# honglu2875/hironaka

Hardware: NVIDIA B200
Metric: game_steps_per_sec (higher is better)
Workload: dtype int32

## Files before the change

### hironaka_b200/csrc/hk_capi.cu

```cuda
#include <cuda_runtime.h>

#include <atomic>
#include <cstdio>
#include <cstring>
#include <new>

#include "hk_experience.cuh"
#include "hk_launch.cuh"
#include "hk_value.cuh"

using hk::StepParams;
using hk::kMaxDevices;

namespace hk {
int launch_small_i32_noobs(const StepParams& p, int dev, cudaStream_t stream);
int launch_small_i32_obs(const StepParams& p, int dev, cudaStream_t stream);
int launch_small_f32_noobs(const StepParams& p, int dev, cudaStream_t stream);
int launch_small_f32_obs(const StepParams& p, int dev, cudaStream_t stream);
int launch_small_i32(const StepParams& p, bool obs, int dev, cudaStream_t stream) {
    return obs ? launch_small_i32_obs(p, dev, stream) : launch_small_i32_noobs(p, dev, stream);
}
int launch_small_f32(const StepParams& p, bool obs, int dev, cudaStream_t stream) {
    return obs ? launch_small_f32_obs(p, dev, stream) : launch_small_f32_noobs(p, dev, stream);
}
// ... 48 lines not shown
        if (nibble && (p.d > 3 || !(p.flags & HK_F_ACT_DISCRETE))) return HK_ERR_BAD_ARG;
        if (host_fixed) p.host_action = nullptr;
        if (agent_fixed || packed) p.axis = nullptr;
        if ((p.ops & HK_OP_SHIFT) &&
            ((!host_fixed && p.host_action == nullptr) || (!agent_fixed && !packed && p.axis == nullptr)))
            return HK_ERR_BAD_ARG;
    }
    if ((p.ops & HK_OP_RESCALE) && dtype != HK_DTYPE_F32) return HK_ERR_UNSUPPORTED;
    if (p.ops & ~(HK_OP_SHIFT | HK_OP_REPOSITION | HK_OP_NEWTON | HK_OP_RESCALE | HK_OP_DEDUPE)) return HK_ERR_BAD_ARG;
    {
        const uint32_t sm = p.flags & (HK_F_OBS_SORT_COORD0 | HK_F_OBS_SORT_LEX | HK_F_OBS_SORT_LEX_FIRST);
        if (sm & (sm - 1)) return HK_ERR_BAD_ARG;
    }
    if (p.T < 1) return HK_ERR_BAD_ARG;
    if (p.B == 0) return HK_OK;
    int dev = 0;
    cudaError_t e = cudaGetDevice(&dev);
    if (e != cudaSuccess) return (int)e;
    const bool obs = p.obs != nullptr;
    if (p.done_bits && !p.census) return HK_ERR_UNSUPPORTED;
    if (p.census) {
        const bool policy = p.flags & (HK_F_HOST_ALL_COORD | HK_F_HOST_ZEILLINGER | HK_F_AGENT_FIRST | HK_F_AGENT_LAST);
        if (p.out != p.in || p.T != 1 || policy || p.host_out || p.ops == 0) return HK_ERR_UNSUPPORTED;
        const bool sched = hk::is_small_shape(p.N, p.d) && !force_generic && !(p.ops & HK_OP_DEDUPE);
        if (obs && !(sched && (p.flags & (HK_F_OBS_SORT_COORD0 | HK_F_OBS_SORT_LEX | HK_F_OBS_SORT_LEX_FIRST))))
            return HK_ERR_UNSUPPORTED;
        if (sched && obs)
            return dtype == HK_DTYPE_I32 ? hk::launch_sched_i32_obs(p, dev, stream) : hk::launch_sched_f32_obs(p, dev, stream);
        if (sched)
            return dtype == HK_DTYPE_I32 ? hk::launch_sched_i32(p, dev, stream) : hk::launch_sched_f32(p, dev, stream);
        if (hk::rows_shape(p.N, p.d) && !(p.ops & HK_OP_DEDUPE) && !g_no_rows_kernel.load()) {
            p.live_mask = reinterpret_cast<uint64_t*>(p.census + ((p.B + 7) & ~7ll));
            int rc2 = dtype == HK_DTYPE_I32 ? hk::launch_rows_i32(p, dev, stream) : hk::launch_rows_f32(p, dev, stream);
            if (rc2 != HK_OK) return rc2;
            p.rows_k = hk::ROWS_K;
        } else if (p.done_bits) {
            e = cudaMemsetAsync(p.done_bits, 0, (size_t)((p.B + 31) / 32) * 4, stream);
            if (e != cudaSuccess) return (int)e;
        }
        return dtype == HK_DTYPE_I32 ? hk::launch_generic_i32(p, false, dev, stream) : hk::launch_generic_f32(p, false, dev, stream);
    }
    const bool small = hk::is_small_shape(p.N, p.d) && !force_generic && !(p.ops & HK_OP_DEDUPE);
    if (dtype == HK_DTYPE_I32)
        return small ? hk::launch_small_i32(p, obs, dev, stream) : hk::launch_generic_i32(p, obs, dev, stream);
    return small ? hk::launch_small_f32(p, obs, dev, stream) : hk::launch_generic_f32(p, obs, dev, stream);
}

StepParams make_params(const void* in, void* out, long long B, int N, int d, float pad) {
    StepParams p;
    memset(&p, 0, sizeof(p));
    p.in = in;
    p.out = out;
    p.B = B;
    p.N = N;
    p.d = d;
// ... 3 lines not shown
    return p;
}

std::atomic<int> g_force_generic{0};
std::atomic<int> g_no_session_graphs{0};

}

namespace hk {
int device_sms(int dev) { return device_sms_impl(dev); }
bool use_pdl() { return g_use_pdl.load(std::memory_order_relaxed) != 0; }
int sched_geometry() { return g_sched_geometry.load(std::memory_order_relaxed); }
}

extern "C" {

int hk_version(void) { return HK_VERSION; }

const char* hk_error_string(int code) {
    switch (code) {
        case HK_OK: return "ok";
        case HK_ERR_BAD_ARG: return "bad argument (null pointer, non-positive size or bad flag combination)";
        case HK_ERR_UNSUPPORTED: return "unsupported shape or op for this dtype";
        case HK_ERR_ALIGN: return "state pointer is not 4-byte aligned";
        default: return code > 0 ? cudaGetErrorString((cudaError_t)code) : "unknown error";
    }
}

int hk_kernel_class(int N, int d) {
    if (check_shape(1, N, d, HK_DTYPE_I32) != HK_OK) return HK_ERR_UNSUPPORTED;
    return (hk::is_small_shape(N, d) && !g_force_generic.load()) ? 1 : 0;
}

int hk_debug_set_pdl(int on) {
    g_use_pdl.store(on ? 1 : 0);
    return HK_OK;
}

int hk_debug_set_sched_geometry(int which) {
    g_sched_geometry.store(which);
    return HK_OK;
}

int hk_debug_set_rows_kernel(int on) {
    g_no_rows_kernel.store(on ? 0 : 1);
    return HK_OK;
}

int64_t hk_census_bytes(int64_t B, int32_t N, int32_t d) {
    if (B < 0) return 0;
    if (hk::is_small_shape(N, d) || !hk::rows_shape(N, d)) return B;
    return ((B + 7) & ~7ll) + 8 * B;
}

int hk_debug_set_session_graphs(int on) {
    g_no_session_graphs.store(on ? 0 : 1);
    return HK_OK;
}

int hk_debug_force_generic(int on) {
    g_force_generic.store(on ? 1 : 0);
    return HK_OK;
}

int hk_step(const void* state_in, void* state_out, const int32_t* host_action, const int32_t* axis, uint8_t* done,
            float* reward, int32_t* num_points, float* obs, const int32_t* obs_coord, int32_t* exceed_flag,
            int64_t B, int32_t N, int32_t d, int32_t dtype, uint32_t ops, uint32_t flags, float padding_value,
            float value_threshold, void* stream) {
    StepParams p = make_params(state_in, state_out, B, N, d, padding_value);
    p.host_action = host_action;
    p.axis = axis;
    p.done = done;
    p.reward = reward;
    p.num_points = num_points;
    p.obs = obs;
// ... 626 lines not shown
```

### hironaka_b200/csrc/hk_launch.cuh

```cuda
#pragma once
#include <cuda_runtime.h>

#include <atomic>
#include <cstring>

#include "hk_common.cuh"

namespace hk {

constexpr int kMaxDevices = 64;

int device_sms(int dev);
bool use_pdl();
int sched_geometry();

struct KernelFacts {
    std::atomic<int> ctas_per_sm[kMaxDevices];
    KernelFacts() {
        for (auto& c : ctas_per_sm) c.store(0);
    }
};

template <typename K>
int kernel_ctas_per_sm(K kernel, KernelFacts& facts, int dev, int threads, size_t smem, cudaError_t* err) {
// ... 6 lines not shown
    }
    e = cudaOccupancyMaxActiveBlocksPerMultiprocessor(&v, kernel, threads, smem);
    if (e != cudaSuccess) {
        *err = e;
        return 0;
    }
    if (v < 1) v = 1;
    facts.ctas_per_sm[dev].store(v, std::memory_order_release);
    return v;
}

inline bool is_small_shape(int N, int d) { return d == 3 && (N == 20 || N == 10 || N == 5); }

int launch_small_i32(const StepParams& p, bool obs, int dev, cudaStream_t stream);
int launch_small_f32(const StepParams& p, bool obs, int dev, cudaStream_t stream);
int launch_sched_i32(const StepParams& p, int dev, cudaStream_t stream);
int launch_sched_f32(const StepParams& p, int dev, cudaStream_t stream);
int launch_sched_i32_obs(const StepParams& p, int dev, cudaStream_t stream);
int launch_sched_f32_obs(const StepParams& p, int dev, cudaStream_t stream);
int launch_rows_i32(const StepParams& p, int dev, cudaStream_t stream);
int launch_rows_f32(const StepParams& p, int dev, cudaStream_t stream);
constexpr int ROWS_K = 8;
inline bool rows_shape(int N, int d) { return N <= 64 && d >= 2 && d <= 5; }
int launch_generic_i32(const StepParams& p, bool obs, int dev, cudaStream_t stream);
int launch_generic_f32(const StepParams& p, bool obs, int dev, cudaStream_t stream);

}
```

### hironaka_b200/csrc/hk_rows.cuh

```cuda
#pragma once
#include "hk_launch.cuh"
#include "hk_small.cuh"

namespace hk {

constexpr int ROWS_MAX_K = ROWS_K;
constexpr int ROWS_ROUND_GAMES = 1024;

template <int D, int WARPS, int STAGES>
struct RowsLayout {
    static constexpr int LANE_WORDS = ROWS_MAX_K * D + 1 - ((ROWS_MAX_K * D) & 1);
    static constexpr int STAGE_WORDS = 32 * LANE_WORDS;
    static constexpr int CLS_WORDS = ROWS_ROUND_GAMES / 4;
    static constexpr int ORDER_WORDS = ROWS_ROUND_GAMES / 2;
    static constexpr int WARP_WORDS = STAGES * STAGE_WORDS + CLS_WORDS + ORDER_WORDS;
    static constexpr size_t SMEM_BYTES = (size_t)WARPS * WARP_WORDS * 4;
};

__device__ __forceinline__ int census_count(uint32_t v) { return (v & 0x80u) ? (int)(v & 1u) : (int)v; }

template <typename T, int D, int K>
__device__ __forceinline__ void rows_step(const StepParams& p, const uint32_t* area, uint32_t* g_state, long long g,
                                          uint64_t mask, int cnt, bool valid, int32_t ha, int32_t ax, int& new_cnt,
                                          uint64_t& new_mask, bool& origin, bool& exceed) {
    T y[K * D];
    uint32_t clm = 0;
#pragma unroll
    for (int k = 0; k < K; ++k) {
        const bool lv = valid && k < cnt;
        clm |= lv ? (1u << k) : 0u;
#pragma unroll
        for (int c = 0; c < D; ++c) y[k * D + c] = lv ? Elem<T>::from_bits(area[k * D + c]) : Elem<T>::zero();
    }
    const uint32_t clm0 = clm;
    clm = game_step<T, K, D, 0, false>(y, clm, p.ops, p.flags, ha, ax);
    new_cnt = __popc(clm);
    if (p.exceed_flag) exceed = exceeds<T, K, D>(y, clm, p.threshold);
    const T padv = Elem<T>::pad(p.pad);
    uint64_t m = mask, nm = mask;
    uint32_t nz = 0;
#pragma unroll
    for (int k = 0; k < K; ++k) {
        if ((clm0 >> k) & 1u) {
            const int slot = __ffsll((long long)m) - 1;
            m &= m - 1;
            const bool alive = (clm >> k) & 1u;
            bool moved = false;
#pragma unroll
            for (int c = 0; c < D; ++c) {
                moved = moved || ((uint32_t)Elem<T>::bits(y[k * D + c]) != area[k * D + c]);
                nz |= alive ? (uint32_t)Elem<T>::bits(y[k * D + c]) : 0u;
            }
            if (!alive) nm &= ~(1ull << slot);
            if (!alive || moved) {
                uint32_t* dst = g_state + slot * D;
#pragma unroll
                for (int c = 0; c < D; ++c) dst[c] = (uint32_t)Elem<T>::bits(alive ? y[k * D + c] : padv);
            }
        }
    }
    new_mask = nm;
    origin = (nz == 0);
}

template <typename T, int D, int WARPS, int STAGES>
__global__ void __launch_bounds__(WARPS * 32) hk_rows_kernel(const StepParams p) {
    using L = RowsLayout<D, WARPS, STAGES>;
    constexpr int LW = L::LANE_WORDS;
    extern __shared__ __align__(128) uint8_t smem_raw[];
    const int warp = threadIdx.x >> 5, lane = threadIdx.x & 31;
    uint32_t* wbase = reinterpret_cast<uint32_t*>(smem_raw) + (size_t)warp * L::WARP_WORDS;
    uint32_t* stages = wbase;
    uint8_t* clsb = reinterpret_cast<uint8_t*>(wbase + STAGES * L::STAGE_WORDS);
    uint16_t* order = reinterpret_cast<uint16_t*>(wbase + STAGES * L::STAGE_WORDS + L::CLS_WORDS);

    const long long B = p.B;
    const int W = p.N * D;
    const long long gw = (long long)blockIdx.x * WARPS + warp;
    const long long nw = (long long)gridDim.x * WARPS;
    uint32_t* gst = reinterpret_cast<uint32_t*>(p.out);
    const uint32_t lt = (1u << lane) - 1u;
    const bool frozen_rest = (p.flags & HK_F_FREEZE_ENDED) && !(p.ops & (HK_OP_REPOSITION | HK_OP_RESCALE));
    const float rest_reward = (p.flags & HK_F_ROLE_AGENT) ? -0.0f : 0.0f;
    int done_total = 0;

    long long per = (B + nw - 1) / nw;
// ... 52 lines not shown
                total += __popc(bal);
            }
        }
        __syncwarp();
        const int nchunks = (total + 31) >> 5;

        struct Pick {
            long long g;
            uint64_t mask;
            int cnt;
            bool valid;
        };
        auto pick = [&](int v) -> Pick {
            Pick k;
            const int idx = v * 32 + lane;
            k.valid = idx < total;
            const int o = k.valid ? (int)order[idx] : 0;
            k.g = g0 + o;
            k.cnt = k.valid ? (int)(clsb[o] >> 2) : 0;
            k.mask = k.valid ? __ldg(reinterpret_cast<const unsigned long long*>(p.live_mask) + k.g) : 0ull;
            return k;
        };
        auto gather = [&](const Pick& k, uint32_t* stage) {
            uint32_t* area = stage + lane * LW;
            const uint32_t* src = gst + k.g * W;
            uint64_t m = k.mask;
#pragma unroll
            for (int r = 0; r < ROWS_MAX_K; ++r) {
                if (r < k.cnt) {
                    const int slot = __ffsll((long long)m) - 1;
                    m &= m - 1;
#pragma unroll
                    for (int c = 0; c < D; ++c) cp_async_4(area + r * D + c, src + slot * D + c);
                }
            }
            cp_async_commit();
        };

        Pick cur = pick(0), nxt;
        nxt.g = 0, nxt.mask = 0, nxt.cnt = 0, nxt.valid = false;
        gather(cur, stages);
        for (int v = 0; v < nchunks; ++v) {
            uint32_t* stage = stages + (STAGES == 1 ? 0 : (v & 1)) * L::STAGE_WORDS;
            int32_t ha = 3, ax = 0;
            if ((p.ops & HK_OP_SHIFT) && cur.valid) load_actions(p, p.flags, cur.g, 0, ha, ax);
            if (STAGES >= 2 && v + 1 < nchunks) {
                nxt = pick(v + 1);
                gather(nxt, stages + ((v + 1) & 1) * L::STAGE_WORDS);
                cp_async_wait<1>();
            } else {
                cp_async_wait<0>();
            }
            __syncwarp();
            const int cmax = __reduce_max_sync(0xffffffffu, cur.cnt);
            const uint32_t* area = stage + lane * LW;
            int ncnt = 0;
            uint64_t nmask = 0;
            bool origin = false, exceed = false;
            const bool prev_done = cur.cnt < 2;
// ... 35 lines not shown
```

### hironaka_b200/csrc/hk_sched.cuh

```cuda
#pragma once
#include "hk_small.cuh"

namespace hk {

constexpr int SCHED_ROUND_TILES = 32;
#ifndef SCHED_PASS_UNROLL
#define SCHED_PASS_UNROLL 2
#endif
constexpr int kSchedPassUnroll = SCHED_PASS_UNROLL;
#ifndef SCHED_TILE_GROUP
#define SCHED_TILE_GROUP 0
#endif
#ifndef SCHED_DIRECT
#define SCHED_DIRECT 1
#endif
#ifndef SCHED_SPECULATE
#define SCHED_SPECULATE 0
#endif
#ifndef SCHED_NATURAL_NUM
#define SCHED_NATURAL_NUM 1
#define SCHED_NATURAL_DEN 2
#endif

template <int N, int D, int WARPS, int STAGES, bool OBS = false>
struct SchedLayout {
    static constexpr int W = N * D;
    static constexpr int STAGE_WORDS = 32 * W;
    static constexpr int OBS_WORDS = OBS ? 32 * (W + D) : 0;
    static constexpr int CLS_WORDS = SCHED_ROUND_TILES * 32 / 4;
    static constexpr int ORDER_WORDS = SCHED_ROUND_TILES * 32 / 2;
    static constexpr int WARP_WORDS = STAGES * STAGE_WORDS + CLS_WORDS + ORDER_WORDS + OBS_WORDS;
    static constexpr int BAR_BYTES = 256;
    static_assert(WARPS * STAGES * 8 <= BAR_BYTES, "mbarrier area too small");
    static constexpr size_t SMEM_BYTES = BAR_BYTES + (size_t)WARPS * WARP_WORDS * 4;
};

__device__ __forceinline__ int census_class(uint32_t v) {
    if (v == 0) return 6;
    if (v & 0x80u) return 1;
    return v <= 2 ? 1 : (v <= 4 ? 2 : (v <= 8 ? 3 : (v <= 12 ? 4 : (v <= 16 ? 5 : 6))));
}

template <typename T, int N, int D, int WARPS, int STAGES, bool OBS = false, int MINB = 1>
__global__ void __launch_bounds__(WARPS * 32, MINB) hk_sched_kernel(const StepParams p) {
    using L = SchedLayout<N, D, WARPS, STAGES, OBS>;
    constexpr int W = L::W;
    constexpr int CHW = (W % 4 == 0) ? 4 : ((W % 2 == 0) ? 2 : 1);
    constexpr int LPG = W / CHW;
    static_assert(LPG <= 32, "a game is copied by at most one warp instruction");
    constexpr int GPI = 32 / LPG;
    constexpr int COPY_ITERS = (32 + GPI - 1) / GPI;
    extern __shared__ __align__(128) uint8_t smem_raw[];
    const int warp = threadIdx.x >> 5, lane = threadIdx.x & 31;
    uint64_t* bar = reinterpret_cast<uint64_t*>(smem_raw) + warp * STAGES;
    uint32_t* wbase = reinterpret_cast<uint32_t*>(smem_raw + L::BAR_BYTES) + (size_t)warp * L::WARP_WORDS;
    uint32_t* stages = wbase;
    uint8_t* clsb = reinterpret_cast<uint8_t*>(wbase + STAGES * L::STAGE_WORDS);
    uint16_t* order = reinterpret_cast<uint16_t*>(wbase + STAGES * L::STAGE_WORDS + L::CLS_WORDS);
    float* obs_tile = reinterpret_cast<float*>(wbase + STAGES * L::STAGE_WORDS + L::CLS_WORDS + L::ORDER_WORDS);
    const int OW = W + (p.obs_coord ? D : 0);
    const bool obs_bulk = OBS && aligned16(p.obs) && ((OW & 3) == 0);

    const long long B = p.B;
    const long long ntiles = (B + 31) >> 5;
    const long long gw = (long long)blockIdx.x * WARPS + warp;
    const long long nw = (long long)gridDim.x * WARPS;
    uint32_t* gst = reinterpret_cast<uint32_t*>(p.out);
    const bool piece_ok = ((reinterpret_cast<uintptr_t>(p.out)) & (CHW * 4 - 1)) == 0;
    const bool bulk = ((W * 4) % 16 == 0) && aligned16(p.out);
    if (lane == 0) {
#pragma unroll
        for (int s = 0; s < STAGES; ++s) mbar_init(&bar[s], 1);
        mbar_fence_init();
    }
    __syncwarp();
    uint32_t phase_bits = 0;
    const uint32_t lt = (1u << lane) - 1u;
    const bool frozen_rest = (p.flags & HK_F_FREEZE_ENDED) && !(p.ops & (HK_OP_REPOSITION | HK_OP_RESCALE));
    const float rest_reward = (p.flags & HK_F_ROLE_AGENT) ? -0.0f : 0.0f;
    const int sub = lane / LPG, piece = lane - sub * LPG;
    int settled_total = 0;

// ... 63 lines not shown
                    fence_async_smem();
                    __syncwarp();
                    if (lane == 0) {
                        mbar_expect_tx(&bar[0], (uint32_t)__popc(vbal) * (uint32_t)(W * 4));
                        bulk_load(stages, gst + first * W, (uint32_t)__popc(vbal) * (uint32_t)(W * 4), &bar[0]);
                    }
                }
            }
            if constexpr (!OBS) {
                if (rest) {
                    if (p.done) p.done[g] = 1;
                    if (p.reward) p.reward[g] = rest_reward;
                    if (p.num_points) p.num_points[g] = (int32_t)(v & 1u);
                }
                const uint32_t restmask = __ballot_sync(0xffffffffu, rest);
                settled_total += __popc(restmask);
                if (p.done_bits && lane == 0) p.done_bits[tile_of(j0 + k)] = restmask;
            }
        }
        classes = __reduce_or_sync(0xffffffffu, classes) & ~1u;
        const bool natural = OBS ? (inplay * 4 >= ngames) : (inplay * SCHED_NATURAL_DEN >= ngames * SCHED_NATURAL_NUM);
        __syncwarp();
        int total = 0;
        if (!natural && inplay <= 32) {
#pragma unroll kSchedPassUnroll
            for (int k = 0; k < nk; ++k) {
                if (!((tilemask >> k) & 1u)) continue;
                const bool m = (clsb[k * 32 + lane] & 7u) != 0u;
                const uint32_t bal = __ballot_sync(0xffffffffu, m);
                if (m) order[total + __popc(bal & lt)] = (uint16_t)(k * 32 + lane);
                total += __popc(bal);
            }
        }
        for (int q = 1; q <= 6 && !natural && inplay > 32; ++q) {
            if (!((classes >> q) & 1u)) continue;
            for (int k = 0; k < nk; ++k) {
                if (!((tilemask >> k) & 1u)) continue;
                const bool m = (clsb[k * 32 + lane] & 7u) == (uint32_t)q;
                const uint32_t bal = __ballot_sync(0xffffffffu, m);
                if (m) order[total + __popc(bal & lt)] = (uint16_t)(k * 32 + lane);
                total += __popc(bal);
            }
        }
        __syncwarp();
        const int nchunks = natural ? __popc(tilemask) : ((total + 31) >> 5);
        uint32_t tiles_left = tilemask;

        auto chunk_game = [&](int v, long long& g, bool& valid) {
            if (natural) {
                const int k = __ffs((int)tiles_left) - 1;
                tiles_left &= tiles_left - 1;
                g = (tile_of(j0 + k) << 5) + lane;
                valid = (g < B) && ((clsb[k * 32 + lane] & 7u) != 0);
                return;
            }
            const int idx = v * 32 + lane;
            valid = idx < total;
// ... 40 lines not shown
                for (int it = 0; it < COPY_ITERS; ++it) {
                    const int s = it * GPI + sub;
                    const long long gs = __shfl_sync(0xffffffffu, g, s & 31);
                    const bool vs = __shfl_sync(0xffffffffu, valid ? 1 : 0, s & 31) != 0;
                    if (sub < GPI && s < 32 && vs) {
                        uint32_t* dst = stage + s * W + piece * CHW;
                        const uint32_t* src = gst + gs * W + piece * CHW;
                        if constexpr (CHW == 4) cp_async_16(dst, src);
                        else if constexpr (CHW == 2) cp_async_8(dst, src);
                        else cp_async_4(dst, src);
                    }
                }
            } else {
                for (int s = 0; s < 32; ++s) {
                    const long long gs = __shfl_sync(0xffffffffu, g, s);
                    const bool vs = __shfl_sync(0xffffffffu, valid ? 1 : 0, s) != 0;
                    if (vs) {
                        for (int w = lane; w < W; w += 32) cp_async_4(stage + s * W + w, gst + gs * W + w);
                    }
                }
            }
            cp_async_commit();
        };

        long long g_cur = 0, g_nxt = 0;
        bool v_cur = false, v_nxt = false;
        if (spec && !natural) {
            mbar_wait(&bar[0], phase_bits & 1u);
            phase_bits ^= 1u;
            spec = false;
        }
        if (inplay) {
            chunk_game(0, g_cur, v_cur);
            if (!spec) gather(g_cur, v_cur, stages, 0);
        }
        for (int k = 0; OBS && k < nk; ++k) {
            const long long g = (tile_of(j0 + k) << 5) + lane;
            const uint32_t code = clsb[k * 32 + lane];
            const bool rest = code & 0x80u;
            const uint32_t v = (code >> 6) & 1u;
            if (rest) {
                if (p.done) p.done[g] = 1;
                if (p.reward) p.reward[g] = rest_reward;
                if (p.num_points) p.num_points[g] = (int32_t)v;
            }
            const uint32_t restmask = __ballot_sync(0xffffffffu, rest);
            settled_total += __popc(restmask);
            if constexpr (OBS) {
                if (p.obs && restmask && !(natural && ((tilemask >> k) & 1u))) {
                    float* orow = obs_tile + lane * OW;
                    bulk_wait_read<0>();
                    __syncwarp();
                    if (rest) {
                        const float z = (v & 1u) ? 0.0f : p.pad;
                        const uint32_t ocm = p.obs_coord ? action_mask(load_action(p.obs_coord, g, p.flags), p.flags) : 0u;
                        if ((OW & 3) == 0 && D <= 4 && !p.obs_coord) {
                            float4* o4 = reinterpret_cast<float4*>(orow);
// ... 26 lines not shown
                            m &= m - 1;
                            warp_copy_words(reinterpret_cast<uint32_t*>(p.obs + (first + r) * OW),
                                            reinterpret_cast<uint32_t*>(obs_tile + r * OW), OW, lane);
                        }
                    }
                    __syncwarp();
                }
            }
            if (p.done_bits && lane == 0) p.done_bits[tile_of(j0 + k)] = restmask;
        }
        __syncwarp();
        if (inplay == 0) continue;
        for (int v = 0; v < nchunks; ++v) {
            const int sidx = (STAGES == 1) ? 0 : (v & 1);
            uint32_t* stage = stages + sidx * L::STAGE_WORDS;
            LaneState ls;
            ls.g = g_cur;
            ls.valid = v_cur;
            ls.shift = (p.ops & HK_OP_SHIFT) && ls.valid;
            ls.ha = 3;
            ls.ax = 0;
            ls.origin = false;
            if (ls.shift) load_actions(p, p.flags, ls.g, 0, ls.ha, ls.ax);
            if constexpr (STAGES == 1 && HK_L2_PREFETCH) {
                if (bulk && natural && tiles_left && lane == 0) {
                    const long long tn = tile_of(j0 + (__ffs((int)tiles_left) - 1));
                    const long long left = B - (tn << 5);
                    bulk_prefetch_l2(gst + (tn << 5) * W, (uint32_t)(left < 32 ? left : 32) * (uint32_t)(W * 4));
                }
            }
            if (bulk) {
                mbar_wait(&bar[sidx], (phase_bits >> sidx) & 1u);
                phase_bits ^= (1u << sidx);
            }
            if constexpr (STAGES >= 2) {
                if (v + 1 < nchunks) {
                    chunk_game(v + 1, g_nxt, v_nxt);
                    gather(g_nxt, v_nxt, stages + ((v + 1) & 1) * L::STAGE_WORDS, (v + 1) & 1);
                    if (!bulk) cp_async_wait<1>();
                } else {
                    if (!bulk) cp_async_wait<0>();
                }
            } else {
                if (!bulk) cp_async_wait<0>();
            }
            __syncwarp();
// ... 1 lines not shown
            bool exceed = false;
            bool chg = false;
            bool released = false;
            if constexpr (SCHED_DIRECT && !OBS && STAGES == 1 && !Elem<T>::is_float) {
                auto release = [&]() {
                    released = true;
                    __syncwarp();
                    if (v + 1 < nchunks) {
                        chunk_game(v + 1, g_nxt, v_nxt);
                        gather(g_nxt, v_nxt, stages, 0);
                    }
                };
                small_process_tile<T, N, D, false, true, decltype(release)>(p, ls, row, exceed, chg, gst + ls.g * W,
                                                                            release);
            } else {
                small_process_tile<T, N, D, false>(p, ls, row, exceed, chg);
            }
            if (ls.valid) {
                if (p.num_points) p.num_points[ls.g] = ls.cnt;
                if (p.done_bits && ls.cnt < 2) atomicOr(p.done_bits + (ls.g >> 5), 1u << (ls.g & 31));
                const uint32_t nv = (ls.cnt <= 1) ? (0x80u | (ls.origin ? 2u : 0u) | (uint32_t)ls.cnt)
                                                  : (uint32_t)(ls.cnt > 127 ? 127 : ls.cnt);
                p.census[ls.g] = (uint8_t)nv;
            }
            if (p.exceed_flag) {
                if (__any_sync(0xffffffffu, exceed && ls.valid) && lane == 0) *p.exceed_flag = 1;
            }
            if constexpr (OBS) {
                if (p.obs) {
                    const bool ingrid = ls.g < B;
                    float* orow = obs_tile + lane * OW;
                    bulk_wait_read<0>();
                    __syncwarp();
                    {
                        T z[W];
                        load_game<T, W>(row, z);
                        if constexpr (Elem<T>::is_float) {
#pragma unroll
                            for (int q = 0; q < W; ++q) z[q] = z[q] + 0.0f;
                        }
                        const uint32_t zl = live_mask<T, N, D>(z);
                        const int zmax = __reduce_max_sync(0xffffffffu, ingrid ? __popc(zl) : 0);
                        bool built = false;
                        if constexpr (D <= 6) built = features_network<T, N, D>(z, zl, zmax, p.flags, p.pad, orow);
                        if (!built) {
                            const int gpow = (OW & -OW) > 32 ? 32 : (OW & -OW);
// ... 103 lines not shown
```

### hironaka_b200/csrc/hk_small.cuh

```cuda
#pragma once
#include <type_traits>

#include "hk_common.cuh"

namespace hk {

constexpr int SMALL_BAR_BYTES = 256;
#ifndef HK_SPARSE_STORE_MAX
#define HK_SPARSE_STORE_MAX 16
#endif

template <int N, int D, bool OBS, int WARPS, int STAGES>
struct SmallLayout {
    static_assert(WARPS * STAGES * 8 <= SMALL_BAR_BYTES, "mbarrier area too small");
    static constexpr int W = N * D;
    static constexpr int TILE_WORDS = 32 * W;
    static constexpr int OBS_W = W + D;
    static constexpr int OBS_WORDS = OBS ? 32 * OBS_W : 0;
    static constexpr int WARP_WORDS = STAGES * TILE_WORDS + OBS_WORDS;
    static constexpr size_t SMEM_BYTES = SMALL_BAR_BYTES + (size_t)WARPS * WARP_WORDS * 4;
};

template <typename T, int W>
__device__ __forceinline__ void load_game(const uint32_t* s, T (&x)[W]) {
// ... 283 lines not shown
            lm = op_newton<T, N, D>(x, lm);
        }
    }
    if constexpr (Elem<T>::is_float) {
        if (ops & HK_OP_RESCALE) op_rescale<N, D>(x, lm, flags & HK_F_RESCALE_EPS);
    }
    return lm;
}

template <typename T>
__device__ __forceinline__ T x_row_value(const uint32_t* row, int w) {
    T v = Elem<T>::from_bits(row[w]);
    if constexpr (Elem<T>::is_float) v = v + 0.0f;
    return v;
}

struct LaneState {
    long long g;
    bool valid, shift;
    int32_t ha, ax;
    int cnt;
    int32_t len;
    bool origin;
};

__host__ __device__ constexpr int next_lower_tier(int K) {
    return K > 16 ? 16 : (K > 12 ? 12 : (K > 8 ? 8 : (K > 4 ? 4 : 0)));
}

template <typename T, int N, int D, int K, bool POLICY>
__device__ __forceinline__ int tier_steps(const StepParams& p, LaneState& ls, uint32_t* row, uint32_t lm, int st,
                                          bool& exceed, bool& chg) {
    const long long B = p.B;
    const T padv = Elem<T>::pad(p.pad);
    const bool mutate = p.ops != 0;
    constexpr bool ROLLED = (K >= 12) && (K < N) && ((N * D) % 4 == 0);
    constexpr int RS = !ROLLED ? 0 : ((D == 3 && 4 * K <= N * D) ? 4 : D);
    constexpr int LOWER = next_lower_tier(K);
    T y[K * D];
    int idx[K];
    uint32_t clm = 0, cvalid = 0;
    if constexpr (K == N) {
        load_game<T, N * D>(row, y);
        if constexpr (Elem<T>::is_float) {
#pragma unroll
            for (int q = 0; q < N * D; ++q) y[q] = y[q] + 0.0f;
// ... 37 lines not shown
        if (ls.valid) {
            if (p.done) p.done[(long long)st * B + ls.g] = dn ? 1 : 0;
            if (p.reward) {
                float r = (dn && !prev_done) ? 1.0f : 0.0f;
                p.reward[(long long)st * B + ls.g] = (p.flags & HK_F_ROLE_AGENT) ? -r : r;
            }
        }
        if (p.done_count) {
            const int c = __popc(__ballot_sync(0xffffffffu, ls.valid && dn));
            if ((threadIdx.x & 31) == 0 && c) atomicAdd(p.done_count + st, c);
        }
        if (dn && !prev_done) ls.len = st + 1;
        ls.ha = ha_n;
        ls.ax = ax_n;
        ++st;
        if constexpr (LOWER > 0) {
            if (st < p.T && __reduce_max_sync(0xffffffffu, ls.valid ? ls.cnt : 0) <= LOWER) break;
        }
    }
    chg = tchg;
    const bool last = st >= p.T;
    if (last && p.exceed_flag) exceed = exceeds<T, K, D>(y, clm, p.threshold);
    if (p.census) {
        if (K <= 4 || __any_sync(0xffffffffu, ls.cnt <= 1)) {
            uint32_t nz = 0;
#pragma unroll
            for (int k = 0; k < K; ++k) {
                uint32_t o = 0;
#pragma unroll
                for (int c = 0; c < D; ++c) o |= (uint32_t)Elem<T>::bits(y[k * D + c]);
                nz |= ((clm >> k) & 1u) ? o : 0u;
            }
            ls.origin = (nz == 0);
        } else {
            ls.origin = false;
        }
    }
    if (mutate) {
        if constexpr (K == N) {
#pragma unroll
            for (int i = 0; i < N; ++i) {
#pragma unroll
                for (int c = 0; c < D; ++c) y[i * D + c] = ((clm >> i) & 1u) ? y[i * D + c] : padv;
            }
            store_game<T, N * D>(row, y);
        } else {
// ... 51 lines not shown
        k[i] = min(a_, b_);                  \
        k[j] = max(a_, b_);                  \
    }
#include "hk_sortnet.inc"
#undef HK_CE
}

template <int D>
struct PackedRow {
    static constexpr int FB = 27 / D;
    static constexpr uint32_t VMAX = (1u << (FB - 1)) - 1u;
    static constexpr uint32_t FMASK = (1u << FB) - 1u;
    __host__ __device__ static constexpr uint32_t guards() {
        uint32_t g = 0;
        for (int c = 0; c < D; ++c) g |= 1u << (5 + FB * c + FB - 1);
        return g;
    }
};

struct NoRelease {
    __device__ __forceinline__ void operator()() const {}
};

template <int N, int D, int K, bool DIRECT = false, typename Release = NoRelease>
__device__ __forceinline__ bool tier_packed(const StepParams& p, LaneState& ls, uint32_t* row, uint32_t lm_in, int lmax, int st,
                                            bool& exceed, bool& chg, uint32_t* gdst = nullptr, Release release = Release()) {
    using P = PackedRow<D>;
    constexpr uint32_t G = P::guards();
    const uint32_t lm = ls.valid ? lm_in : 0u;
    const int cnt0 = __popc(lm);
    uint32_t M[D], csel[D];
    const int ax = ls.ax;
    bool apply = false;
    {
        uint32_t cm = 0;
        if (p.ops & HK_OP_SHIFT) {
            cm = action_mask(ls.ha, p.flags);
            apply = (ax >= 0) && (ax < D);
            if (p.flags & HK_F_NOOP_INVALID) apply = apply && ((cm >> (ax & 31)) & 1u);
            if (p.flags & HK_F_FREEZE_ENDED) apply = apply && (cnt0 >= 2);
        }
        const uint32_t into = apply ? (1u << (5 + P::FB * ax)) : 0u;
#pragma unroll
        for (int c = 0; c < D; ++c) {
            csel[c] = apply ? ((cm >> c) & 1u) : 0u;
            M[c] = ((apply && c == ax) ? 0u : (1u << (5 + P::FB * c))) + csel[c] * into;
        }
    }
    constexpr int KLOW = (K > 16) ? 16 : ((K > 12) ? 12 : (K > 8 ? 8 : (K > 4 ? 4 : 0)));
    uint32_t w[K];
    uint32_t uor = 0, orig0 = 0, orig_hi = 0;
    uint32_t mn[D], mns = 0xffffffffu;
#pragma unroll
    for (int c = 0; c < D; ++c) mn[c] = 0xffffffffu;
    {
        uint32_t m = lm;
        int i = 0;
        uint32_t pa[D], ps = 0xffffffffu;
#pragma unroll
        for (int c = 0; c < D; ++c) pa[c] = 0xffffffffu;
#pragma unroll
        for (int k = 0; k < K; ++k) {
            if (k >= KLOW && k >= lmax) {
                w[k] = 0xffffffffu;
                continue;
            }
            const bool v = m != 0;
            i = v ? (__ffs((int)m) - 1) : i;
            m &= m - 1;
            uint32_t a[D];
#pragma unroll
            for (int c = 0; c < D; ++c) a[c] = row[i * D + c];
            if (k == 0) {
#pragma unroll
                for (int c = 0; c < D; ++c) {
                    orig0 += a[c] << (5 + P::FB * c);
                    orig_hi |= a[c];
                }
            }
            uint32_t q = (uint32_t)i, sum = 0;
#pragma unroll
            for (int c = 0; c < D; ++c) {
                q += a[c] * M[c];
                sum += a[c] * csel[c];
                uor |= a[c];
            }
            uor |= sum;
            if (k & 1) {
#pragma unroll
                for (int c = 0; c < D; ++c) mn[c] = __vimin3_u32(mn[c], pa[c], a[c]);
                mns = __vimin3_u32(mns, ps, sum);
            } else {
#pragma unroll
                for (int c = 0; c < D; ++c) pa[c] = a[c];
                ps = sum;
// ... 26 lines not shown
            for (int a = 0; a + 1 < b; a += 2) acc = __vimin3_u32(acc, ~(pb - w[a]) & G, ~(pb - w[a + 1]) & G);
            if (b & 1) acc = min(acc, ~(pb - w[b - 1]) & G);
            kill |= (acc == 0u) ? (1u << b) : 0u;
        }
    }
    const uint32_t live0 = (cnt0 >= 32) ? 0xffffffffu : ((1u << cnt0) - 1u);
    const uint32_t alive = live0 & ~kill;
    const int cnt = __popc(alive);
    const bool prev_done = cnt0 < 2, dn = cnt < 2;
    if (ls.valid) {
        if (p.done) p.done[(long long)st * p.B + ls.g] = dn ? 1 : 0;
        if (p.reward) {
            const float r = (dn && !prev_done) ? 1.0f : 0.0f;
            p.reward[(long long)st * p.B + ls.g] = (p.flags & HK_F_ROLE_AGENT) ? -r : r;
        }
    }
    if (p.done_count) {
        const int c = __popc(__ballot_sync(0xffffffffu, ls.valid && dn));
        if ((threadIdx.x & 31) == 0 && c) atomicAdd(p.done_count + st, c);
    }
    if (dn && !prev_done) ls.len = st + 1;
    ls.cnt = cnt;
    ls.origin = (cnt == 0) || (cnt == 1 && (w[0] >> 5) == 0u);
    const bool gchg = (cnt0 >= 2) || (cnt0 == 1 && lone_moved);
    if constexpr (!DIRECT) chg = chg || gchg;
    if (p.exceed_flag && st + 1 >= p.T) {
        uint32_t hi = 0;
#pragma unroll
        for (int b = 0; b < K; ++b) {
#pragma unroll
            for (int c = 0; c < D; ++c) hi = ((alive >> b) & 1u) ? max(hi, (w[b] >> (5 + P::FB * c)) & P::VMAX) : hi;
        }
        exceed = (cnt > 0) && ((float)hi >= p.threshold);
    }
    const uint32_t padw = (uint32_t)(int32_t)p.pad;
#pragma unroll
    for (int b = 0; b < K; ++b) {
        if (b < lmax) {
            if (gchg && b < cnt0) {
                const bool lv = (alive >> b) & 1u;
                const int i = (int)(w[b] & 31u);
                uint32_t* dst = DIRECT ? (gdst + i * D) : (row + i * D);
                if constexpr (DIRECT && D == 3 && HK_DIRECT_PAIR_STORES) {
                    uint32_t v[3];
#pragma unroll
                    for (int c = 0; c < 3; ++c) v[c] = lv ? ((w[b] >> (5 + P::FB * c)) & P::FMASK) : padw;
                    const bool ev = ((reinterpret_cast<uintptr_t>(dst) >> 2) & 1u) == 0;
                    *reinterpret_cast<uint2*>(dst + (ev ? 0 : 1)) = ev ? make_uint2(v[0], v[1]) : make_uint2(v[1], v[2]);
                    dst[ev ? 2 : 0] = ev ? v[2] : v[0];
                } else {
#pragma unroll
                    for (int c = 0; c < D; ++c) dst[c] = lv ? ((w[b] >> (5 + P::FB * c)) & P::FMASK) : padw;
                }
            }
        }
    }
    return true;
}

template <int N>
__device__ __forceinline__ void sort_keys_desc(uint32_t (&k)[N]) {
#define HK_CE(i, j)                   \
    {                                 \
        const uint32_t a_ = k[i], b_ = k[j]; \
        k[i] = max(a_, b_);           \
        k[j] = min(a_, b_);           \
    }
#include "hk_sortnet.inc"
#undef HK_CE
}

template <typename T, int N, int D>
__device__ __forceinline__ bool features_network(const T (&z)[N * D], uint32_t lm, int zmax, uint32_t flags, float padf,
                                                 float* orow) {
    static_assert(N <= 31 && D >= 2 && D <= 6, "5 tag bits, at least 4 bits per coordinate");
    constexpr int W = N * D;
    constexpr int BITS = 27 / D;
    constexpr uint32_t FMASK = (1u << BITS) - 1u;
    const bool sorted = flags & (HK_F_OBS_SORT_COORD0 | HK_F_OBS_SORT_LEX | HK_F_OBS_SORT_LEX_FIRST);
    const bool lex = flags & HK_F_OBS_SORT_LEX;
// ... 334 lines not shown
#pragma unroll
                        for (int q = 0; q < W; ++q) x[q] = x[q] + 0.0f;
                    }
#pragma unroll
                    for (int i = 0; i < N; ++i) {
#pragma unroll
                        for (int c = 0; c < D; ++c) x[i * D + c] = ((lm >> i) & 1u) ? x[i * D + c] : padv;
                    }
                    store_game<T, W>(row, x);
                }
                normalised = true;
            }
        };
        constexpr bool HAS_PACKED = HK_PACKED_TIERS && PACKED && !Elem<T>::is_float && !POLICY && D == 3;
        if constexpr (HAS_PACKED) {
            if ((p.ops & HK_OP_NEWTON) && lmax <= 20 &&
                ((p.T == 1 && lmax >= HK_PACKED_MIN) || (HK_PACKED_ROLLOUT && p.T > 1 && lmax >= 2))) {
                prestore();
                int32_t ha_n = 3, ax_n = 0;
                if (ls.shift && st + 1 < p.T) load_actions(p, p.flags, ls.g, st + 1, ha_n, ax_n);
                bool ok = false, tried = false;
                if constexpr (!std::is_same<Release, NoRelease>::value) {
                    if (gdst != nullptr && p.T == 1 && lmax <= HK_DIRECT_MAX_ROWS && !any_junk && !__any_sync(0xffffffffu, chg)) {
                        if (lmax <= 4) ok = tier_packed<N, D, 4, true, Release>(p, ls, row, lm, lmax, st, exceed, chg, gdst, release);
#if HK_DIRECT_MAX_ROWS > 8
                        else if (lmax > 8) ok = tier_packed<N, D, 12, true, Release>(p, ls, row, lm, lmax, st, exceed, chg, gdst, release);
#endif
                        else ok = tier_packed<N, D, 8, true, Release>(p, ls, row, lm, lmax, st, exceed, chg, gdst, release);
                        if (ok) return true;
                        tried = true;
                    }
                }
                if (!tried) {
                    if (lmax <= 4) ok = tier_packed<N, D, 4>(p, ls, row, lm, lmax, st, exceed, chg);
                    else if (lmax <= 8) ok = tier_packed<N, D, 8>(p, ls, row, lm, lmax, st, exceed, chg);
                    else if (lmax <= 12) ok = tier_packed<N, D, 12>(p, ls, row, lm, lmax, st, exceed, chg);
                    else if (N <= 16 || lmax <= 16) ok = tier_packed<N, D, 16>(p, ls, row, lm, lmax, st, exceed, chg);
                    else ok = tier_packed<N, D, (N > 16 ? 20 : 16)>(p, ls, row, lm, lmax, st, exceed, chg);
                }
                if (ok) {
                    ls.ha = ha_n;
                    ls.ax = ax_n;
                    ++st;
                    continue;
                }
            }
        }
        if (N > 2 && p.T == 1 && lmax <= 2) {
            prestore();
            st = tier_steps<T, N, D, (N > 2 ? 2 : N), POLICY>(p, ls, row, lm, st, exceed, chg);
        } else if (N > 4 && lmax <= 4) {
            prestore();
            st = tier_steps<T, N, D, (N > 4 ? 4 : N), POLICY>(p, ls, row, lm, st, exceed, chg);
        } else if (N > 8 && lmax <= 8) {
            prestore();
            st = tier_steps<T, N, D, (N > 8 ? 8 : N), POLICY>(p, ls, row, lm, st, exceed, chg);
        } else if (N > 12 && lmax <= 12) {
            if (W % 4 != 0) prestore();
            st = tier_steps<T, N, D, (N > 12 ? 12 : N), POLICY>(p, ls, row, lm, st, exceed, chg);
            normalised = normalised || (W % 4 == 0);
        } else if (N > 16 && lmax <= 16) {
// ... 219 lines not shown
```

Baseline: 24.01 billion.

## Gather only live rows via census masks in the small-shape scheduler

Census calls for small shapes now maintain a per-game 64-bit live-point mask, and the scheduler kernel uses it to cp.async only the live rows of chunks where every game has few points. Those games are stepped on a compact row area with double-buffered prefetch of the next chunk. This replaces the full-game gather for nearly finished games, reducing global memory traffic. The cost is an extra mask load and a mask store on every stepped game, a more complex pipeline, and a new 8-byte alignment requirement on the census buffer.

```diff
diff --git a/hironaka_b200/csrc/hk_capi.cu b/hironaka_b200/csrc/hk_capi.cu
--- a/hironaka_b200/csrc/hk_capi.cu
+++ b/hironaka_b200/csrc/hk_capi.cu
@@ -94,6 +94,11 @@
     if (p.census) {
         const bool policy = p.flags & (HK_F_HOST_ALL_COORD | HK_F_HOST_ZEILLINGER | HK_F_AGENT_FIRST | HK_F_AGENT_LAST);
         if (p.out != p.in || p.T != 1 || policy || p.host_out || p.ops == 0) return HK_ERR_UNSUPPORTED;
+        if (hk::census_has_masks(p.N, p.d)) {
+            uint8_t* masks = p.census + hk::census_mask_offset(p.B);
+            if ((uintptr_t)masks & 7u) return HK_ERR_ALIGN;
+            p.live_mask = reinterpret_cast<uint64_t*>(masks);
+        }
         const bool sched = hk::is_small_shape(p.N, p.d) && !force_generic && !(p.ops & HK_OP_DEDUPE);
         if (obs && !(sched && (p.flags & (HK_F_OBS_SORT_COORD0 | HK_F_OBS_SORT_LEX | HK_F_OBS_SORT_LEX_FIRST))))
             return HK_ERR_UNSUPPORTED;
@@ -102,7 +107,6 @@
         if (sched)
             return dtype == HK_DTYPE_I32 ? hk::launch_sched_i32(p, dev, stream) : hk::launch_sched_f32(p, dev, stream);
         if (hk::rows_shape(p.N, p.d) && !(p.ops & HK_OP_DEDUPE) && !g_no_rows_kernel.load()) {
-            p.live_mask = reinterpret_cast<uint64_t*>(p.census + ((p.B + 7) & ~7ll));
             int rc2 = dtype == HK_DTYPE_I32 ? hk::launch_rows_i32(p, dev, stream) : hk::launch_rows_f32(p, dev, stream);
             if (rc2 != HK_OK) return rc2;
             p.rows_k = hk::ROWS_K;
@@ -152,7 +156,7 @@
         case HK_OK: return "ok";
         case HK_ERR_BAD_ARG: return "bad argument (null pointer, non-positive size or bad flag combination)";
         case HK_ERR_UNSUPPORTED: return "unsupported shape or op for this dtype";
-        case HK_ERR_ALIGN: return "state pointer is not 4-byte aligned";
+        case HK_ERR_ALIGN: return "state pointer is not 4-byte aligned, or the live masks of a census are not 8-byte aligned";
         default: return code > 0 ? cudaGetErrorString((cudaError_t)code) : "unknown error";
     }
 }
@@ -179,8 +183,8 @@
 
 int64_t hk_census_bytes(int64_t B, int32_t N, int32_t d) {
     if (B < 0) return 0;
-    if (hk::is_small_shape(N, d) || !hk::rows_shape(N, d)) return B;
-    return ((B + 7) & ~7ll) + 8 * B;
+    if (!hk::census_has_masks(N, d)) return B;
+    return hk::census_mask_offset(B) + 8 * B;
 }
 
 int hk_debug_set_session_graphs(int on) {
diff --git a/hironaka_b200/csrc/hk_launch.cuh b/hironaka_b200/csrc/hk_launch.cuh
--- a/hironaka_b200/csrc/hk_launch.cuh
+++ b/hironaka_b200/csrc/hk_launch.cuh
@@ -52,6 +52,8 @@
 int launch_rows_f32(const StepParams& p, int dev, cudaStream_t stream);
 constexpr int ROWS_K = 8;
 inline bool rows_shape(int N, int d) { return N <= 64 && d >= 2 && d <= 5; }
+inline bool census_has_masks(int N, int d) { return rows_shape(N, d); }
+inline long long census_mask_offset(long long B) { return (B + 7) & ~7ll; }
 int launch_generic_i32(const StepParams& p, bool obs, int dev, cudaStream_t stream);
 int launch_generic_f32(const StepParams& p, bool obs, int dev, cudaStream_t stream);
 
diff --git a/hironaka_b200/csrc/hk_rows.cuh b/hironaka_b200/csrc/hk_rows.cuh
--- a/hironaka_b200/csrc/hk_rows.cuh
+++ b/hironaka_b200/csrc/hk_rows.cuh
@@ -9,59 +9,13 @@
 
 template <int D, int WARPS, int STAGES>
 struct RowsLayout {
-    static constexpr int LANE_WORDS = ROWS_MAX_K * D + 1 - ((ROWS_MAX_K * D) & 1);
+    static constexpr int LANE_WORDS = compact_lane_words(ROWS_MAX_K, D);
     static constexpr int STAGE_WORDS = 32 * LANE_WORDS;
     static constexpr int CLS_WORDS = ROWS_ROUND_GAMES / 4;
     static constexpr int ORDER_WORDS = ROWS_ROUND_GAMES / 2;
     static constexpr int WARP_WORDS = STAGES * STAGE_WORDS + CLS_WORDS + ORDER_WORDS;
     static constexpr size_t SMEM_BYTES = (size_t)WARPS * WARP_WORDS * 4;
 };
-
-__device__ __forceinline__ int census_count(uint32_t v) { return (v & 0x80u) ? (int)(v & 1u) : (int)v; }
-
-template <typename T, int D, int K>
-__device__ __forceinline__ void rows_step(const StepParams& p, const uint32_t* area, uint32_t* g_state, long long g,
-                                          uint64_t mask, int cnt, bool valid, int32_t ha, int32_t ax, int& new_cnt,
-                                          uint64_t& new_mask, bool& origin, bool& exceed) {
-    T y[K * D];
-    uint32_t clm = 0;
-#pragma unroll
-    for (int k = 0; k < K; ++k) {
-        const bool lv = valid && k < cnt;
-        clm |= lv ? (1u << k) : 0u;
-#pragma unroll
-        for (int c = 0; c < D; ++c) y[k * D + c] = lv ? Elem<T>::from_bits(area[k * D + c]) : Elem<T>::zero();
-    }
-    const uint32_t clm0 = clm;
-    clm = game_step<T, K, D, 0, false>(y, clm, p.ops, p.flags, ha, ax);
-    new_cnt = __popc(clm);
-    if (p.exceed_flag) exceed = exceeds<T, K, D>(y, clm, p.threshold);
-    const T padv = Elem<T>::pad(p.pad);
-    uint64_t m = mask, nm = mask;
-    uint32_t nz = 0;
-#pragma unroll
-    for (int k = 0; k < K; ++k) {
-        if ((clm0 >> k) & 1u) {
-            const int slot = __ffsll((long long)m) - 1;
-            m &= m - 1;
-            const bool alive = (clm >> k) & 1u;
-            bool moved = false;
-#pragma unroll
-            for (int c = 0; c < D; ++c) {
-                moved = moved || ((uint32_t)Elem<T>::bits(y[k * D + c]) != area[k * D + c]);
-                nz |= alive ? (uint32_t)Elem<T>::bits(y[k * D + c]) : 0u;
-            }
-            if (!alive) nm &= ~(1ull << slot);
-            if (!alive || moved) {
-                uint32_t* dst = g_state + slot * D;
-#pragma unroll
-                for (int c = 0; c < D; ++c) dst[c] = (uint32_t)Elem<T>::bits(alive ? y[k * D + c] : padv);
-            }
-        }
-    }
-    new_mask = nm;
-    origin = (nz == 0);
-}
 
 template <typename T, int D, int WARPS, int STAGES>
 __global__ void __launch_bounds__(WARPS * 32) hk_rows_kernel(const StepParams p) {
@@ -160,19 +114,7 @@
             return k;
         };
         auto gather = [&](const Pick& k, uint32_t* stage) {
-            uint32_t* area = stage + lane * LW;
-            const uint32_t* src = gst + k.g * W;
-            uint64_t m = k.mask;
-#pragma unroll
-            for (int r = 0; r < ROWS_MAX_K; ++r) {
-                if (r < k.cnt) {
-                    const int slot = __ffsll((long long)m) - 1;
-                    m &= m - 1;
-#pragma unroll
-                    for (int c = 0; c < D; ++c) cp_async_4(area + r * D + c, src + slot * D + c);
-                }
-            }
-            cp_async_commit();
+            gather_live_rows<D, ROWS_MAX_K>(stage + lane * LW, gst + k.g * W, k.mask, k.cnt);
         };
 
         Pick cur = pick(0), nxt;
diff --git a/hironaka_b200/csrc/hk_sched.cuh b/hironaka_b200/csrc/hk_sched.cuh
--- a/hironaka_b200/csrc/hk_sched.cuh
+++ b/hironaka_b200/csrc/hk_sched.cuh
@@ -41,6 +41,39 @@
     return v <= 2 ? 1 : (v <= 4 ? 2 : (v <= 8 ? 3 : (v <= 12 ? 4 : (v <= 16 ? 5 : 6))));
 }
 
+template <typename T, int N, int D>
+__device__ __forceinline__ void sched_row_step(const StepParams& p, LaneState& ls, const uint32_t* area, uint32_t mask,
+                                               uint32_t* game, bool& exceed) {
+    const int cnt0 = __popc(mask);
+    const int lmax = __reduce_max_sync(0xffffffffu, cnt0);
+    bool chg = false;
+    if ((p.ops & HK_OP_NEWTON) && lmax >= HK_PACKED_MIN) {
+        const bool ok = (lmax <= 4) ? tier_packed<N, D, 4, true>(p, ls, CompactRows<D>{area}, mask, lmax, 0, exceed, chg, game)
+                                    : tier_packed<N, D, 8, true>(p, ls, CompactRows<D>{area}, mask, lmax, 0, exceed, chg, game);
+        if (ok) return;
+    }
+    int cnt = 0;
+    uint64_t nm = 0;
+    bool origin = false;
+    if (lmax <= 4) rows_step<T, D, 4>(p, area, game, ls.g, mask, cnt0, ls.valid, ls.ha, ls.ax, cnt, nm, origin, exceed);
+    else rows_step<T, D, 8>(p, area, game, ls.g, mask, cnt0, ls.valid, ls.ha, ls.ax, cnt, nm, origin, exceed);
+    const bool prev_done = cnt0 < 2, dn = cnt < 2;
+    if (ls.valid) {
+        if (p.done) p.done[ls.g] = dn ? 1 : 0;
+        if (p.reward) {
+            const float r = (dn && !prev_done) ? 1.0f : 0.0f;
+            p.reward[ls.g] = (p.flags & HK_F_ROLE_AGENT) ? -r : r;
+        }
+    }
+    if (p.done_count) {
+        const int c = __popc(__ballot_sync(0xffffffffu, ls.valid && dn));
+        if ((threadIdx.x & 31) == 0 && c) atomicAdd(p.done_count, c);
+    }
+    ls.cnt = cnt;
+    ls.origin = origin;
+    ls.lmask = (uint32_t)nm;
+}
+
 template <typename T, int N, int D, int WARPS, int STAGES, bool OBS = false, int MINB = 1>
 __global__ void __launch_bounds__(WARPS * 32, MINB) hk_sched_kernel(const StepParams p) {
     using L = SchedLayout<N, D, WARPS, STAGES, OBS>;
@@ -58,6 +91,9 @@
     uint8_t* clsb = reinterpret_cast<uint8_t*>(wbase + STAGES * L::STAGE_WORDS);
     uint16_t* order = reinterpret_cast<uint16_t*>(wbase + STAGES * L::STAGE_WORDS + L::CLS_WORDS);
     float* obs_tile = reinterpret_cast<float*>(wbase + STAGES * L::STAGE_WORDS + L::CLS_WORDS + L::ORDER_WORDS);
+    constexpr int ROW_K = 8;
+    constexpr int RLW = compact_lane_words(ROW_K, D);
+    constexpr bool ROW_ROUTE = SCHED_DIRECT && !OBS && STAGES == 1 && !Elem<T>::is_float && D == 3 && 2 * 32 * RLW <= L::STAGE_WORDS;
     const int OW = W + (p.obs_coord ? D : 0);
     const bool obs_bulk = OBS && aligned16(p.obs) && ((OW & 3) == 0);
 
@@ -167,6 +203,7 @@
         const bool natural = OBS ? (inplay * 4 >= ngames) : (inplay * SCHED_NATURAL_DEN >= ngames * SCHED_NATURAL_NUM);
         __syncwarp();
         int total = 0;
+        int nsmall = 0;
         if (!natural && inplay <= 32) {
 #pragma unroll kSchedPassUnroll
             for (int k = 0; k < nk; ++k) {
@@ -176,8 +213,10 @@
                 if (m) order[total + __popc(bal & lt)] = (uint16_t)(k * 32 + lane);
                 total += __popc(bal);
             }
+            nsmall = (classes >> 4) ? 0 : total;
         }
         for (int q = 1; q <= 6 && !natural && inplay > 32; ++q) {
+            if (q == 4) nsmall = total;
             if (!((classes >> q) & 1u)) continue;
             for (int k = 0; k < nk; ++k) {
                 if (!((tilemask >> k) & 1u)) continue;
@@ -264,17 +303,34 @@
             }
             cp_async_commit();
         };
+        auto row_chunk = [&](int v) -> bool {
+            return ROW_ROUTE && !natural && ((v * 32 + 32 < total) ? (v * 32 + 32) : total) <= nsmall;
+        };
+        auto fetch = [&](int v, long long& g, bool& valid, uint32_t& m) {
+            chunk_game(v, g, valid);
+            if (row_chunk(v)) {
+                m = valid ? (uint32_t)__ldg(reinterpret_cast<const unsigned long long*>(p.live_mask) + g) : 0u;
+                if (bulk) {
+                    bulk_wait_read<0>();
+                    __syncwarp();
+                }
+                gather_live_rows<D, ROW_K>(stages + (v & 1) * 32 * RLW + lane * RLW, gst + g * W, m, __popc(m));
+            } else {
+                gather(g, valid, stages, 0);
+            }
+        };
 
         long long g_cur = 0, g_nxt = 0;
         bool v_cur = false, v_nxt = false;
+        uint32_t m_cur = 0, m_nxt = 0;
         if (spec && !natural) {
             mbar_wait(&bar[0], phase_bits & 1u);
             phase_bits ^= 1u;
             spec = false;
         }
         if (inplay) {
-            chunk_game(0, g_cur, v_cur);
-            if (!spec) gather(g_cur, v_cur, stages, 0);
+            if (!spec) fetch(0, g_cur, v_cur, m_cur);
+            else chunk_game(0, g_cur, v_cur);
         }
         for (int k = 0; OBS && k < nk; ++k) {
             const long long g = (tile_of(j0 + k) << 5) + lane;
@@ -347,6 +403,35 @@
             ls.ax = 0;
             ls.origin = false;
             if (ls.shift) load_actions(p, p.flags, ls.g, 0, ls.ha, ls.ax);
+            if constexpr (ROW_ROUTE) {
+                if (row_chunk(v)) {
+                    const uint32_t* area = stages + (v & 1) * 32 * RLW + lane * RLW;
+                    if (v + 1 < nchunks && row_chunk(v + 1)) {
+                        fetch(v + 1, g_nxt, v_nxt, m_nxt);
+                        cp_async_wait<1>();
+                    } else {
+                        cp_async_wait<0>();
+                    }
+                    __syncwarp();
+                    bool exceed = false;
+                    sched_row_step<T, N, D>(p, ls, area, m_cur, gst + ls.g * W, exceed);
+                    if (ls.valid) {
+                        if (p.num_points) p.num_points[ls.g] = ls.cnt;
+                        if (p.done_bits && ls.cnt < 2) atomicOr(p.done_bits + (ls.g >> 5), 1u << (ls.g & 31));
+                        p.census[ls.g] = (uint8_t)((ls.cnt <= 1) ? (0x80u | (ls.origin ? 2u : 0u) | (uint32_t)ls.cnt) : (uint32_t)ls.cnt);
+                        if (ls.lmask != m_cur) p.live_mask[ls.g] = ls.lmask;
+                    }
+                    if (p.exceed_flag) {
+                        if (__any_sync(0xffffffffu, exceed && ls.valid) && lane == 0) *p.exceed_flag = 1;
+                    }
+                    __syncwarp();
+                    if (v + 1 < nchunks && !row_chunk(v + 1)) fetch(v + 1, g_nxt, v_nxt, m_nxt);
+                    g_cur = g_nxt;
+                    v_cur = v_nxt;
+                    m_cur = m_nxt;
+                    continue;
+                }
+            }
             if constexpr (STAGES == 1 && HK_L2_PREFETCH) {
                 if (bulk && natural && tiles_left && lane == 0) {
                     const long long tn = tile_of(j0 + (__ffs((int)tiles_left) - 1));
@@ -394,6 +479,7 @@
                 const uint32_t nv = (ls.cnt <= 1) ? (0x80u | (ls.origin ? 2u : 0u) | (uint32_t)ls.cnt)
                                                   : (uint32_t)(ls.cnt > 127 ? 127 : ls.cnt);
                 p.census[ls.g] = (uint8_t)nv;
+                p.live_mask[ls.g] = ls.lmask;
             }
             if (p.exceed_flag) {
                 if (__any_sync(0xffffffffu, exceed && ls.valid) && lane == 0) *p.exceed_flag = 1;
diff --git a/hironaka_b200/csrc/hk_small.cuh b/hironaka_b200/csrc/hk_small.cuh
--- a/hironaka_b200/csrc/hk_small.cuh
+++ b/hironaka_b200/csrc/hk_small.cuh
@@ -329,6 +329,7 @@
     int cnt;
     int32_t len;
     bool origin;
+    uint32_t lmask;
 };
 
 __host__ __device__ constexpr int next_lower_tier(int K) {
@@ -412,6 +413,14 @@
     const bool last = st >= p.T;
     if (last && p.exceed_flag) exceed = exceeds<T, K, D>(y, clm, p.threshold);
     if (p.census) {
+        if constexpr (K == N) {
+            ls.lmask = clm;
+        } else {
+            uint32_t nm = 0;
+#pragma unroll
+            for (int k = 0; k < K; ++k) nm |= ((clm >> k) & 1u) ? (1u << idx[k]) : 0u;
+            ls.lmask = nm;
+        }
         if (K <= 4 || __any_sync(0xffffffffu, ls.cnt <= 1)) {
             uint32_t nz = 0;
 #pragma unroll
@@ -509,8 +518,19 @@
     __device__ __forceinline__ void operator()() const {}
 };
 
-template <int N, int D, int K, bool DIRECT = false, typename Release = NoRelease>
-__device__ __forceinline__ bool tier_packed(const StepParams& p, LaneState& ls, uint32_t* row, uint32_t lm_in, int lmax, int st,
+template <int D>
+struct SlotRows {
+    uint32_t* row;
+    __device__ __forceinline__ uint32_t at(int, int i, int c) const { return row[i * D + c]; }
+};
+template <int D>
+struct CompactRows {
+    const uint32_t* area;
+    __device__ __forceinline__ uint32_t at(int k, int, int c) const { return area[k * D + c]; }
+};
+
+template <int N, int D, int K, bool DIRECT = false, typename Release = NoRelease, typename Rows = SlotRows<D>>
+__device__ __forceinline__ bool tier_packed(const StepParams& p, LaneState& ls, const Rows& rows, uint32_t lm_in, int lmax, int st,
                                             bool& exceed, bool& chg, uint32_t* gdst = nullptr, Release release = Release()) {
     using P = PackedRow<D>;
     constexpr uint32_t G = P::guards();
@@ -542,7 +562,7 @@
     for (int c = 0; c < D; ++c) mn[c] = 0xffffffffu;
     {
         uint32_t m = lm;
-        int i = 0;
+        int i = 0, kl = 0;
         uint32_t pa[D], ps = 0xffffffffu;
 #pragma unroll
         for (int c = 0; c < D; ++c) pa[c] = 0xffffffffu;
@@ -554,10 +574,11 @@
             }
             const bool v = m != 0;
             i = v ? (__ffs((int)m) - 1) : i;
+            kl = v ? k : kl;
             m &= m - 1;
             uint32_t a[D];
 #pragma unroll
-            for (int c = 0; c < D; ++c) a[c] = row[i * D + c];
+            for (int c = 0; c < D; ++c) a[c] = rows.at(kl, i, c);
             if (k == 0) {
 #pragma unroll
                 for (int c = 0; c < D; ++c) {
@@ -630,6 +651,12 @@
     if (dn && !prev_done) ls.len = st + 1;
     ls.cnt = cnt;
     ls.origin = (cnt == 0) || (cnt == 1 && (w[0] >> 5) == 0u);
+    if (p.census) {
+        uint32_t nm = 0;
+#pragma unroll
+        for (int b = 0; b < K; ++b) nm |= (b < lmax && ((alive >> b) & 1u)) ? (1u << (w[b] & 31u)) : 0u;
+        ls.lmask = nm;
+    }
     const bool gchg = (cnt0 >= 2) || (cnt0 == 1 && lone_moved);
     if constexpr (!DIRECT) chg = chg || gchg;
     if (p.exceed_flag && st + 1 >= p.T) {
@@ -648,7 +675,9 @@
             if (gchg && b < cnt0) {
                 const bool lv = (alive >> b) & 1u;
                 const int i = (int)(w[b] & 31u);
-                uint32_t* dst = DIRECT ? (gdst + i * D) : (row + i * D);
+                uint32_t* dst;
+                if constexpr (DIRECT) dst = gdst + i * D;
+                else dst = rows.row + i * D;
                 if constexpr (DIRECT && D == 3 && HK_DIRECT_PAIR_STORES) {
                     uint32_t v[3];
 #pragma unroll
@@ -664,6 +693,68 @@
         }
     }
     return true;
+}
+
+__device__ __forceinline__ int census_count(uint32_t v) { return (v & 0x80u) ? (int)(v & 1u) : (int)v; }
+
+__host__ __device__ constexpr int compact_lane_words(int K, int D) { return K * D + 1 - ((K * D) & 1); }
+
+template <int D, int K>
+__device__ __forceinline__ void gather_live_rows(uint32_t* area, const uint32_t* game, uint64_t mask, int cnt) {
+#pragma unroll
+    for (int r = 0; r < K; ++r) {
+        if (r < cnt) {
+            const int slot = __ffsll((long long)mask) - 1;
+            mask &= mask - 1;
+#pragma unroll
+            for (int c = 0; c < D; ++c) cp_async_4(area + r * D + c, game + slot * D + c);
+        }
+    }
+    cp_async_commit();
+}
+
+template <typename T, int D, int K>
+__device__ __forceinline__ void rows_step(const StepParams& p, const uint32_t* area, uint32_t* g_state, long long g,
+                                          uint64_t mask, int cnt, bool valid, int32_t ha, int32_t ax, int& new_cnt,
+                                          uint64_t& new_mask, bool& origin, bool& exceed) {
+    T y[K * D];
+    uint32_t clm = 0;
+#pragma unroll
+    for (int k = 0; k < K; ++k) {
+        const bool lv = valid && k < cnt;
+        clm |= lv ? (1u << k) : 0u;
+#pragma unroll
+        for (int c = 0; c < D; ++c) y[k * D + c] = lv ? Elem<T>::from_bits(area[k * D + c]) : Elem<T>::zero();
+    }
+    const uint32_t clm0 = clm;
+    clm = game_step<T, K, D, 0, false>(y, clm, p.ops, p.flags, ha, ax);
+    new_cnt = __popc(clm);
+    if (p.exceed_flag) exceed = exceeds<T, K, D>(y, clm, p.threshold);
+    const T padv = Elem<T>::pad(p.pad);
+    uint64_t m = mask, nm = mask;
+    uint32_t nz = 0;
+#pragma unroll
+    for (int k = 0; k < K; ++k) {
+        if ((clm0 >> k) & 1u) {
+            const int slot = __ffsll((long long)m) - 1;
+            m &= m - 1;
+            const bool alive = (clm >> k) & 1u;
+            bool moved = false;
+#pragma unroll
+            for (int c = 0; c < D; ++c) {
+                moved = moved || ((uint32_t)Elem<T>::bits(y[k * D + c]) != area[k * D + c]);
+                nz |= alive ? (uint32_t)Elem<T>::bits(y[k * D + c]) : 0u;
+            }
+            if (!alive) nm &= ~(1ull << slot);
+            if (!alive || moved) {
+                uint32_t* dst = g_state + slot * D;
+#pragma unroll
+                for (int c = 0; c < D; ++c) dst[c] = (uint32_t)Elem<T>::bits(alive ? y[k * D + c] : padv);
+            }
+        }
+    }
+    new_mask = nm;
+    origin = (nz == 0);
 }
 
 template <int N>
@@ -1044,21 +1135,21 @@
                 bool ok = false, tried = false;
                 if constexpr (!std::is_same<Release, NoRelease>::value) {
                     if (gdst != nullptr && p.T == 1 && lmax <= HK_DIRECT_MAX_ROWS && !any_junk && !__any_sync(0xffffffffu, chg)) {
-                        if (lmax <= 4) ok = tier_packed<N, D, 4, true, Release>(p, ls, row, lm, lmax, st, exceed, chg, gdst, release);
+                        if (lmax <= 4) ok = tier_packed<N, D, 4, true, Release>(p, ls, SlotRows<D>{row}, lm, lmax, st, exceed, chg, gdst, release);
 #if HK_DIRECT_MAX_ROWS > 8
-                        else if (lmax > 8) ok = tier_packed<N, D, 12, true, Release>(p, ls, row, lm, lmax, st, exceed, chg, gdst, release);
+                        else if (lmax > 8) ok = tier_packed<N, D, 12, true, Release>(p, ls, SlotRows<D>{row}, lm, lmax, st, exceed, chg, gdst, release);
 #endif
-                        else ok = tier_packed<N, D, 8, true, Release>(p, ls, row, lm, lmax, st, exceed, chg, gdst, release);
+                        else ok = tier_packed<N, D, 8, true, Release>(p, ls, SlotRows<D>{row}, lm, lmax, st, exceed, chg, gdst, release);
                         if (ok) return true;
                         tried = true;
                     }
                 }
                 if (!tried) {
-                    if (lmax <= 4) ok = tier_packed<N, D, 4>(p, ls, row, lm, lmax, st, exceed, chg);
-                    else if (lmax <= 8) ok = tier_packed<N, D, 8>(p, ls, row, lm, lmax, st, exceed, chg);
-                    else if (lmax <= 12) ok = tier_packed<N, D, 12>(p, ls, row, lm, lmax, st, exceed, chg);
-                    else if (N <= 16 || lmax <= 16) ok = tier_packed<N, D, 16>(p, ls, row, lm, lmax, st, exceed, chg);
-                    else ok = tier_packed<N, D, (N > 16 ? 20 : 16)>(p, ls, row, lm, lmax, st, exceed, chg);
+                    if (lmax <= 4) ok = tier_packed<N, D, 4>(p, ls, SlotRows<D>{row}, lm, lmax, st, exceed, chg);
+                    else if (lmax <= 8) ok = tier_packed<N, D, 8>(p, ls, SlotRows<D>{row}, lm, lmax, st, exceed, chg);
+                    else if (lmax <= 12) ok = tier_packed<N, D, 12>(p, ls, SlotRows<D>{row}, lm, lmax, st, exceed, chg);
+                    else if (N <= 16 || lmax <= 16) ok = tier_packed<N, D, 16>(p, ls, SlotRows<D>{row}, lm, lmax, st, exceed, chg);
+                    else ok = tier_packed<N, D, (N > 16 ? 20 : 16)>(p, ls, SlotRows<D>{row}, lm, lmax, st, exceed, chg);
                 }
                 if (ok) {
                     ls.ha = ha_n;
```

Result: slower. 23.62 billion, median of 6 (-1.6%).
